# RemoteSensingTools/vSmartMOM.jl

Hardware: AMD Instinct MI355X
Metric: spectral-points/s (whole node) for rt_run, O2-A band (higher is better)
Workload: dtype f64; 1 GPU; C2: O2-A 759-770 nm, nStokes=3, Nquad=20 (N=60), 40 layers, 10000 spectral points/GPU, m=0..2, Rayleigh+synthetic O2 absorption, Lambertian 0.15; ranks=1, collective_backend=none (1 rank), N=60, layers=40, points_per_gpu=10000, fourier_moments=3

## Files before the change

include/vsmartmom_hip.h:

```cpp
#ifndef VSMARTMOM_HIP_H
#define VSMARTMOM_HIP_H

#include <stddef.h>
#include <stdint.h>

#ifdef __cplusplus
extern "C" {
#endif

typedef enum vsm_status {
  VSM_OK = 0,
  VSM_ERR_INVALID_ARG = 1,
  VSM_ERR_UNSUPPORTED = 2,
  VSM_ERR_HIP = 3,
  VSM_ERR_NO_DEVICE = 4
} vsm_status;

typedef enum vsm_iface {
  VSM_IFACE_00 = 0,
  VSM_IFACE_01 = 1,
  VSM_IFACE_10 = 2,
  VSM_IFACE_11 = 3
} vsm_iface;

// ... 392 lines not shown
                      const double* F0, int ncomp, const double* const* Zpp, const double* const* Zmp, long long z_stride,
                      const double* fcomp, int toa, const int* layer_coupling_h, void* stream);
int vsm_run_layer_f32(vsm_run* run, int ndoubl, const float* dtau, const float* varpi, const float* tau_sum,
                      const float* F0, int ncomp, const float* const* Zpp, const float* const* Zmp, long long z_stride,
                      const float* fcomp, int toa, const int* layer_coupling_h, void* stream);
int vsm_run_export_f64(vsm_run* run, const vsm_composite_f64* comps, void* stream);
int vsm_run_export_f32(vsm_run* run, const vsm_composite_f32* comps, void* stream);
int vsm_run_import_f64(vsm_run* run, const vsm_composite_f64* comps, void* stream);
int vsm_run_import_f32(vsm_run* run, const vsm_composite_f32* comps, void* stream);
int vsm_run_zw_tail(vsm_run* run);
int vsm_run_view_rows(vsm_run* run, int nrows, const int* rows_h);
int vsm_run_view_block(const vsm_run* run, int block, int* im, int* n, int* nv, int* local_rows);
int vsm_run_view_rows(vsm_run* run, int nrows, const int* rows_h);
int vsm_run_view_block(const vsm_run* run, int block, int* im, int* n, int* nv, int* local_rows);
int vsm_run_destroy(vsm_run* run);
int vsm_stokes_coupling_f64(int N, int n_stokes, int nblocks, const double* Zpp, const double* Zmp, int* mask_d, void* stream);
int vsm_stokes_coupling_f32(int N, int n_stokes, int nblocks, const float* Zpp, const float* Zmp, int* mask_d, void* stream);

typedef struct vsm_added_rs_f64 {
  double *ier_mp, *iet_pp, *ier_pm, *iet_mm;
  double *ieJ0_p, *ieJ0_m;
  int K;
  int reserved;
} vsm_added_rs_f64;
typedef struct vsm_added_rs_f32 {
  float *ier_mp, *iet_pp, *ier_pm, *iet_mm;
  float *ieJ0_p, *ieJ0_m;
  int K;
  int reserved;
} vsm_added_rs_f32;
// ... 243 lines not shown
```

vsmartmom.jl_amd/_lib.py:

```python
from __future__ import annotations

import ctypes as C
import os

_HERE = os.path.dirname(os.path.abspath(__file__))
LIB_PATH = os.environ.get("VSM_LIB_PATH") or os.path.join(_HERE, "lib", "libvsmartmom_hip.so")


class VSMError(RuntimeError):
    pass


class vsm_quad_f64(C.Structure):
    _fields_ = [("mu", C.c_void_p), ("wt", C.c_void_p), ("N", C.c_int), ("n_stokes", C.c_int),
                ("i_mu0", C.c_int), ("mu0", C.c_double)]


class vsm_quad_f32(C.Structure):
    _fields_ = [("mu", C.c_void_p), ("wt", C.c_void_p), ("N", C.c_int), ("n_stokes", C.c_int),
                ("i_mu0", C.c_int), ("mu0", C.c_float)]


class vsm_added(C.Structure):
    _fields_ = [("r_mp", C.c_void_p), ("t_pp", C.c_void_p), ("r_pm", C.c_void_p), ("t_mm", C.c_void_p),
# ... 127 lines not shown
    "vsm_exact_ss_jac12_{T}": (_I, [_I, _I, _I, _I, _I, _P, _P, _P, _P, _I, _P, "{R}", _P, _P, _P, _P, _P, _P, _P]),
    "vsm_run_supported": (_I, [_I, _I, _I]),
    "vsm_run_workspace_bytes": (_SZ, [_I, _I, _I, _I, _P]),
    "vsm_run_supported_f32": (_I, [_I, _I, _I]),
    "vsm_run_workspace_bytes_f32": (_SZ, [_I, _I, _I, _I, _P]),
    "vsm_run_create_{T}": (_I, [_P, _I, _I, _P, _P, _P, _SZ, _P]),
    "vsm_run_create_ex_{T}": (_I, [_P, _I, _I, _P, _P, _P, _SZ, C.c_uint, _P]),
    "vsm_run_create_view_{T}": (_I, [_P, _I, _I, _P, _P, _P, _SZ, C.c_uint, _I, _P, _P]),
    "vsm_run_layer_{T}": (_I, [_P, _I, _P, _P, _P, _P, _I, _P, _P, _LL, _P, _I, _P, _P]),
    "vsm_run_export_{T}": (_I, [_P, _P, _P]),
    "vsm_run_import_{T}": (_I, [_P, _P, _P]),
    "vsm_run_zw_tail": (_I, [_P]),
    "vsm_run_view_rows": (_I, [_P, _I, _P]),
    "vsm_run_view_block": (_I, [_P, _I, _P, _P, _P, _P]),
    "vsm_run_destroy": (_I, [_P]),
    "vsm_stokes_coupling_{T}": (_I, [_I, _I, _I, _P, _P, _P, _P]),
    "vsm_level_radiance_work_elems": (_SZ, [_I, _I]),
    "vsm_level_radiance_{T}": (_I, [_I, _I, _I, _I, _P, _P, _P, _P, _P, _LL, _P, _P, _P, _P, _P, _P, _P]),
    "vsm_level_radiance_oplevel_{T}": (_I, [_I, _I, _I, _I, _P, _P, _P, _P, _P, _LL, _P, _P, _P, _P, _P, _P, _P]),
    "vsm_level_radiance_src_{T}": (_I, [_I, _I, _I, _I, _P, _P, _P, _I, _P, _P, _LL, _P, _P, _P, _P, _P, _P, _P]),
    "vsm_level_flux_{T}": (_I, [_I, _I, _I, _P, _I, _P, _P, _LL, _P, _I, _P, _P, "{R}", _P, _P, _P, _P]),
    "vsm_surface_emission_response_{T}": (_I, [_I, _I, _I, _I, _P, _I, _P, _P, _P, _P, _P, _LL, _P, _P, _P]),
    "vsm_level_radiance_ie_{T}": (_I, [_I, _I, _I, _I, _P, _I, _P, _P, _P, _P, _LL, _P, _P, _P, _P, _P, _P, _P, _P, _P, _P, _P]),
    "vsm_level_flux_ie_{T}": (_I, [_I, _I, _I, _I, _P, _P, _P, _LL, _P, _P, _P, _P, _P, _P, _I, _P, _P, "{R}", _P, _P, _P, _P]),
    "vsm_level_radiance_lin_{T}": (_I, [_I, _I, _I, _I, _I, _I, _P, _P, _P, _P, _LL, _P, _P, _P, _LL, _P, _P, _LL, _LL, _P, _P, _P, _P, _P,
                                        _P]),
    "vsm_level_radiance_lin_src_{T}": (_I, [_I, _I, _I, _I, _I, _I, _I, _P, _P, _P, _P, _LL, _P, _P, _P, _LL, _P, _P, _LL, _LL, _P, _P, _P,
                                            _P, _P, _P, _P, _P]),
    "vsm_level_flux_lin_{T}": (_I, [_I, _I, _I, _I, _I, _I, _P, _P, _LL, _P, _P, _P, _LL, _P, _P, _LL, _LL, _P, _P, _P, _I, _P, _P,
                                    "{R}", _P, _P, _P, _I, _P, _P]),
# ... 102 lines not shown
```

vsmartmom.jl_amd/core_rt.py:

```python
from __future__ import annotations

import contextlib
import ctypes as C
import dataclasses
import math
import os
import warnings
from dataclasses import dataclass
from typing import List, Optional

import numpy as np
import torch

from . import _lib
from . import host_model as H
from .architectures import GPU, CPU, architecture, array_type, devi, synchronize_if_gpu, to_host

IFACE = {"00": 0, "01": 1, "10": 2, "11": 3}
MOMENT_BATCH = 4
MOMENT_BATCH_MAX = 24
MOMENT_BATCHING = True
THERMAL_FUSION = True
NATIVE_RUN = True
NATIVE_SOURCES_ONLY = True
NATIVE_VIEW_ROWS = True
VIEW_ROWS_MAX = 16
NATIVE_ZW_TAIL = True
NATIVE_DROPIN = True
REFERENCE_ORDER = False


def _require_gpu(arch):
    if not isinstance(arch, GPU):
        raise _lib.VSMError("vsmartmom.jl_amd provides the MI355X path only; architecture %r has no compute path here "
                            "(no CPU fallback by design)" % (arch,))
    if not torch.cuda.is_available():
        raise _lib.VSMError("no MI355X visible to HIP (torch.cuda.is_available() is False)")
    if arch.device_index != torch.cuda.current_device():
        raise _lib.VSMError("architecture GPU(%d) is not the current HIP device (%d): one process per GPU -- call "
                            "torch.cuda.set_device(%d) first" % (arch.device_index, torch.cuda.current_device(),
                                                                 arch.device_index))

# ... 90 lines not shown
        self.d_symmetric = int(d_symmetric)
        self.r_pm, self.t_mm = (None, None) if self.d_symmetric else (z(), z())
        self.j0_p = torch.zeros((nSpec, N), dtype=dt, device=dev)
        self.j0_m = torch.zeros((nSpec, N), dtype=dt, device=dev)
        self.N, self.nSpec, self.shared, self.dtype = N, nSpec, shared, dt

    def cstruct(self):
        return _lib.vsm_added(self.r_mp.data_ptr(), self.t_pp.data_ptr(),
                              0 if self.r_pm is None else self.r_pm.data_ptr(),
                              0 if self.t_mm is None else self.t_mm.data_ptr(),
                              self.j0_p.data_ptr(), self.j0_m.data_ptr(), 0 if self.shared else self.N * self.N,
                              self.d_symmetric, 0)


def _composite_field(name):
    def fget(self):
        return self.materialize()._arr[name]

    def fset(self, value):
        self.materialize()._arr[name] = value
    return property(fget, fset)


class CompositeLayer:

    def __init__(self, FT, arch, N, nSpec):
        dev, dt = devi(arch), _torch_dtype(FT)
        z = lambda: torch.zeros((nSpec, N, N), dtype=dt, device=dev)
        self._native = None
        self._sources_only = False
        self._view_rows = None
        self._native_ws = None
        self._arr = dict(R_mp=z(), R_pm=z(), T_pp=z(), T_mm=z(), J0_p=torch.zeros((nSpec, N), dtype=dt, device=dev),
                         J0_m=torch.zeros((nSpec, N), dtype=dt, device=dev))
        self.N, self.nSpec, self.dtype = N, nSpec, dt

    R_mp, R_pm, T_pp = _composite_field("R_mp"), _composite_field("R_pm"), _composite_field("T_pp")
    T_mm, J0_p, J0_m = _composite_field("T_mm"), _composite_field("J0_p"), _composite_field("J0_m")

    def materialize(self):
        slot = self._native
        if slot is None:
            return self
        self._native = None
        try:
            cc = (_lib.vsm_composite * 1)(self._cstruct_raw())
            _lib.call("vsm_run_export", self.dtype, slot.run, cc, _stream_ptr())
        finally:
            _lib.lib().vsm_run_destroy(slot.run)
        return self

    def snapshot_top(self):
        slot = self._native
        if slot is not None:
            cc = (_lib.vsm_composite * 1)(self._cstruct_raw())
            _lib.call("vsm_run_export", self.dtype, slot.run, cc, _stream_ptr())
            a = self._arr
        else:
            a = self.materialize()._arr
        return a["R_pm"].clone(), a["J0_p"].clone()

    def drop_native(self):
        slot, self._native = self._native, None
        if slot is not None:
            _lib.lib().vsm_run_destroy(slot.run)

    def _cstruct_raw(self):
        a = self._arr
        return _lib.vsm_composite(a["R_mp"].data_ptr(), a["R_pm"].data_ptr(), a["T_pp"].data_ptr(), a["T_mm"].data_ptr(),
                                  a["J0_p"].data_ptr(), a["J0_m"].data_ptr())

    def cstruct(self):
        self.materialize()
        return self._cstruct_raw()

    def __del__(self):
        try:
            self.drop_native()
        except Exception:
            pass


def make_added_layer(FT, arch, dims, nSpec, shared=False, d_symmetric=0) -> AddedLayer:
    _require_gpu(arch)
    return AddedLayer(FT, arch, dims[0], nSpec, shared, d_symmetric)


def make_composite_layer(FT, arch, dims, nSpec) -> CompositeLayer:
    _require_gpu(arch)
# ... 149 lines not shown
def reflectance(surf, dq: DeviceQuad, m: int, arch, FT, deriv: bool = False):
    if isinstance(surf, (H.rpvSurfaceScalar, H.RossLiSurfaceScalar)):
        if deriv:
            raise _lib.VSMError("%s has no linearization (types.jl:472-512)" % type(surf).__name__)
        return to_device_matrix(H.brdf_reflectance(surf, dq.n_stokes, dq.host.qp_mu.astype(np.float64), m), arch, FT)[0].contiguous(), None
    N = int(dq.mu.numel())
    rho = torch.empty((N, N), dtype=dq.dtype, device=dq.mu.device)
    drho = torch.empty_like(rho) if deriv else None
    phi, w = brdf_azimuth_quadrature(arch, FT)
    cs, q = _coxmunk_cstruct(surf, dq.dtype), dq.cstruct()
    _lib.call("vsm_coxmunk_reflectance", dq.dtype, C.byref(cs), C.byref(q), m, int(phi.numel()), _ptr(phi), _ptr(w), _ptr(rho),
              _ptr(drho), _stream_ptr())
    return rho, drho


def create_surface_layer_(surface, added_surface: AddedLayer, m: int, dq: DeviceQuad, tau_sum: torch.Tensor, rho=None,
                          arch=None, FT=None):
    q, a = dq.cstruct(), added_surface.cstruct()
    if isinstance(surface, (H.LambertianSurfaceLegendre, H.LambertianSurfaceSpline)):
        if added_surface.shared or rho is None:
            raise _lib.VSMError("spectral Lambertian surfaces need a per-point surface AddedLayer and their albedo spectrum")
        _lib.call("vsm_lambertian_surface_spectral", added_surface.dtype, C.byref(q), added_surface.nSpec, m, _ptr(rho),
                  _ptr(tau_sum), C.byref(a), _stream_ptr())
        return
    if not added_surface.shared:
        raise _lib.VSMError("surface AddedLayer must be allocated with shared=True")
    if isinstance(surface, H.LambertianSurfaceScalar):
        surface = surface.albedo
    if isinstance(surface, (int, float)):
        alb = C.c_double(surface) if added_surface.dtype == torch.float64 else C.c_float(surface)
        _lib.call("vsm_lambertian_surface", added_surface.dtype, C.byref(q), added_surface.nSpec, m, alb, _ptr(tau_sum),
                  C.byref(a), _stream_ptr())
        return
    if isinstance(surface, BRDF_SURFACES):
        if rho is None:
            rho, _ = reflectance(surface, dq, m, arch, FT)
        _lib.call("vsm_brdf_surface", added_surface.dtype, C.byref(q), added_surface.nSpec, m, _ptr(rho), _ptr(tau_sum),
                  C.byref(a), _stream_ptr())
        return
    raise _lib.VSMError("surface %r is not built in this backend (LambertianSurfaceScalar / Legendre / Spline, CoxMunkSurface, "
                        "rpvSurfaceScalar, RossLiSurfaceScalar)"
                        % (surface,))


SIF_SURFACES = (H.LambertianSurfaceScalar, H.LambertianSurfaceLegendre, H.LambertianSurfaceSpline)


def surface_source_contribute_(scene_or_table, surface, added_surface: AddedLayer, m: int) -> bool:
    scene = scene_or_table if isinstance(scene_or_table, Scene) else None
    table = scene.sif if scene is not None else scene_or_table
    if table is None or m != 0:
        return False
    if not isinstance(surface, SIF_SURFACES + (int, float)):
        if scene is None or not scene._sif_warned:
# ... 57 lines not shown
        for k in range(n):
            w[v + nV * k] = weight * [c, c, s, s][k]
    return row0, w


def postprocessing_vza_(pol: H.PolarizationType, comp: CompositeLayer, vza, vaz, qp: H.QuadPoints, m: int, weight: float,
                        R_SFI: torch.Tensor, T_SFI: torch.Tensor):
    n, nV = pol.n, len(vza)
    row0, w = _vza_rows_weights(pol, vza, vaz, qp, m, weight, comp.dtype)
    _lib.call("vsm_postprocess_vza", comp.dtype, comp.N, n, comp.nSpec, nV, row0, w, _ptr(comp.J0_m), _ptr(comp.J0_p),
              _ptr(R_SFI), _ptr(T_SFI), _stream_ptr())


def interaction_hdrf_(pol, comp: CompositeLayer, added_surface: AddedLayer, m: int, dq: DeviceQuad, vza, vaz, qp, weight: float,
                      hdr_J: torch.Tensor, hdr: torch.Tensor, bhr_uw: torch.Tensor, bhr_dw: torch.Tensor):
    q, c, a = dq.cstruct(), comp.cstruct(), added_surface.cstruct()
    _lib.call("vsm_interaction_hdrf", comp.dtype, C.byref(q), comp.nSpec, m, C.byref(c), C.byref(a), _ptr(hdr_J), _ptr(bhr_uw),
              _ptr(bhr_dw), _stream_ptr())
    row0, w = _vza_rows_weights(pol, vza, vaz, qp, m, weight, comp.dtype)
    _lib.call("vsm_postprocess_vza_hdrf", comp.dtype, comp.N, pol.n, comp.nSpec, len(vza), row0, w, _ptr(hdr_J), _ptr(hdr),
              _stream_ptr())


def init_layer(props: DeviceLayerOptics, qp: H.QuadPoints, FT, numerics: H.RTNumericalParameters, arch):
    dtau_h, nd = H.get_dtau_ndoubl(props.tau_h, props.varpi_h, qp, FT, numerics)
    return array_type(arch)(dtau_h), nd


@dataclass
class NativeSlot:
    run: C.c_void_p
    m: int
    coupling: int
    grp_of: List[int]


def stokes_groups(n_stokes: int, coupling: int) -> List[int]:
    adj = [[a == b or coupling < 0 or bool((coupling >> (4 * a + b)) & 1) or bool((coupling >> (4 * b + a)) & 1)
            for b in range(n_stokes)] for a in range(n_stokes)]
    grp = [-1] * n_stokes
    ng = 0
    for a in range(n_stokes):
        if grp[a] >= 0:
            continue
        grp[a], stack = ng, [a]
        while stack:
            x = stack.pop()
            for b in range(n_stokes):
                if adj[x][b] and grp[b] < 0:
# ... 53 lines not shown
    nbytes = run_workspace_bytes(comp.dtype, N, ns, S, 1, carr)
    ws = comp._native_ws
    if ws is None or ws.numel() * 8 < nbytes:
        ws = comp._native_ws = _lib.poison(torch.empty(max(nbytes // 8, 2), dtype=torch.float64, device=comp._arr["R_mp"].device))
    q = dq.cstruct()
    comp._native_q = (q, dq)
    run = C.c_void_p()
    run_create_(comp.dtype, q, S, 1, marr, carr, ws, nbytes, comp._sources_only, comp._view_rows, run)
    if import_arrays:
        try:
            cc = (_lib.vsm_composite * 1)(comp._cstruct_raw())
            _lib.call("vsm_run_import", comp.dtype, run, cc, _stream_ptr())
        except Exception:
            L.vsm_run_destroy(run)
            raise
    comp._native = NativeSlot(run, int(m), int(mask), stokes_groups(ns, mask))
    return True


def _rt_kernel_native(comp: CompositeLayer, props: DeviceLayerOptics, tau_sum, m: int, dq: DeviceQuad, iz: int, F0, dtau,
                      ndoubl: int) -> bool:
    N, ns, S = comp.N, dq.n_stokes, comp.nSpec
    ncomp = 0 if props.fcomp is None else int(props.fcomp.shape[1])
    if ncomp > 4 or S == 0:
        return False
    lc = layer_coupling(props, N, ns)
    if iz == 1:
        comp.drop_native()
        if not _native_open(comp, dq, m, lc, False):
            return False
    slot = comp._native
# ... 293 lines not shown
    def _layer_coupling(self, m, iz):
        mixed, k = self.zcomp[iz]
        row = self.coupling_comp[m]
        return int(np.bitwise_or.reduce(row)) if mixed else int(row[k])

    def run(self, trace: Optional[list] = None, streams: Optional[list] = None):
        model, pol, FT = self.model, self.pol, self.FT
        if self.layers_only:
            raise _lib.VSMError("Scene(layers_only=True) holds no composite layer: it feeds rt_run_ss only")
        self.R_SFI.zero_()
        self.T_SFI.zero_()
        self.hdr.zero_()
        if self.S == 0:
            return self.R_SFI, self.T_SFI
        self.added.j0_p.zero_()
        eps2 = 2 * np.finfo(FT).eps
        has_noscat = any(ly["props"].max_tau_varpi <= eps2 for ly in self.moments[0]["layers"])
        nb = self._group_size(trace is not None or not MOMENT_BATCHING or has_noscat or REFERENCE_ORDER)
        native = self._native_moments() if trace is None and not has_noscat and not REFERENCE_ORDER else set()
        walk_src = streams is None and trace is None and not has_noscat
        if getattr(self, "_view_rows", None) is None:
            self._view_rows = view_rows_of(pol, model.vza, self.qp)
        view_rows = self._view_rows if streams is None else None
        with self._walk_composites(nb, walk_src and REFERENCE_ORDER, view_rows):
            for g0 in range(0, len(self.moments), nb):
                group = self.moments[g0:g0 + nb]
                comps = self._composites[:len(group)]
                self._walk_layers(group, comps, [k for k in range(len(group)) if (g0 + k) in native], sources_only=streams is None,
                                  view_rows=view_rows, trace=trace, keep_added=has_noscat)
                for mom, comp in zip(group, comps):
                    m = mom["m"]
                    weight = float(fourier_weight(FT, m))
                    create_surface_layer_(model.surface, self.added_surface, m, self.dq, mom["tau_sum_surface"], rho=mom["rho"])
                    surface_source_contribute_(self, model.surface, self.added_surface, m)
                    interaction_(mom["iface_surface"], comp, self.added_surface, work=self.work)
                    if self.compute_hdrf:
                        interaction_hdrf_(pol, comp, self.added_surface, m, self.dq, model.vza, model.vaz, self.qp, weight,
                                          self.hdr_J, self.hdr, self.bhr_uw, self.bhr_dw)
                    postprocessing_vza_(pol, comp, model.vza, model.vaz, self.qp, m, weight, self.R_SFI, self.T_SFI)
                    thermal_pass = self.thermal_B is not None and (m == 0 or (m == 1 and self.thermal_slot().carry))
                    if thermal_pass:
                        self._thermal_slot(mom, weight)
                    if streams is not None:
                        Jm, Jp = comp.J0_m.clone(), comp.J0_p.clone()
                        if thermal_pass:
                            Jm += self._thermal.comp.J0_m
                            Jp += self._thermal.comp.J0_p
                        streams.append(dict(m=m, weight=weight, R_mp=comp.R_mp.clone(), T_pp=comp.T_pp.clone(), J0_m=Jm, J0_p=Jp))
        if isinstance(model.surface, H.CoxMunkSurface) and self.ss_correction:
            apply_ss_correction_(self.R_SFI, model.surface, pol, model.vza, model.vaz, self.qp.mu0,
                                 self.moments[-1]["tau_sum_surface"], model.m_max, self.arch, FT)
        return self.R_SFI, self.T_SFI

    def _group_size(self, sequential: bool) -> int:
        want = max(MOMENT_BATCH, min(MOMENT_BATCH_MAX, 4096 // max(self.S, 1)))
        return 1 if sequential else min(want, len(self.moments))

    @contextlib.contextmanager
    def _walk_composites(self, nb: int, sources_only: bool, view_rows):
        while len(self._composites) < nb:
            self._composites.append(make_composite_layer(self.FT, self.arch, (self.N, self.N), self.S))
        for c in self._composites:
            c._sources_only = bool(sources_only)
            c._view_rows = view_rows if sources_only else None
        try:
            yield
        finally:
            for c in self._composites:
                c._sources_only = False
                c._view_rows = None

    def _walk_layers(self, group, comps, nat, sources_only: bool, view_rows, trace=None, keep_added: bool = False, tops_at=(),
                     keep_top=None):
        eps2 = 2 * np.finfo(self.FT).eps
        if nat:
            def export(l):
                def cb(cs):
                    for k, c in zip(nat, cs):
                        keep_top(k, l, (c._arr["R_pm"].clone(), c._arr["J0_p"].clone()))
                return cb
            self._run_layers_native([group[k] for k in nat], [comps[k] for k in nat], sources_only=sources_only,
                                    export_at={l: export(l) for l in tops_at}, view_rows=view_rows)
        rest = [k for k in range(len(group)) if k not in nat]
        group_l, comps_l = [group[k] for k in rest], [comps[k] for k in rest]
        for iz in range(self.Nz if rest else 0):
            ly0 = group_l[0]["layers"][iz]
            if len(group_l) > 1 and ly0["props"].max_tau_varpi > eps2 and (iz == 0 or ly0["iface"] == "11"):
                layer_forward_multi_(ly0["tau_sum"], ly0["dtau"], self.F0, [mom["layers"][iz]["props"] for mom in group_l],
                                     [mom["m"] for mom in group_l], ly0["nd"], self.dq, iz == 0, comps_l, self.added)
            else:
                for mom, comp in zip(group_l, comps_l):
                    ly = mom["layers"][iz]
                    rt_kernel_(self.pol, self.added, comp, ly["props"], ly["iface"], ly["tau_sum"], mom["m"], self.dq, self.arch,
                               iz + 1, self.F0, self.FT, self.model.numerics, dtau=ly["dtau"], ndoubl=ly["nd"], trace=trace,
                               work=self.work, keep_added=keep_added)
            if iz + 1 in tops_at:
                for k, comp in zip(rest, comps_l):
                    keep_top(k, iz + 1, comp.snapshot_top())

    def _native_moments(self):
        if not NATIVE_RUN or getattr(self, "coupling", None) is None or not self.moments:
            return set()
        eps2 = 2 * np.finfo(self.FT).eps
        for iz, ly in enumerate(self.moments[0]["layers"]):
            p = ly["props"]
            if p.max_tau_varpi <= eps2 or (iz > 0 and ly["iface"] != "11") or (p.fcomp is not None and p.fcomp.shape[1] > 4):
                return set()
        return {i for i, mom in enumerate(self.moments) if run_supported(self.dt, self.N, self.pol.n, int(self.coupling[mom["m"]]))}

    def _run_layers_native(self, group, comps, sources_only: bool = True, export_at=None, view_rows=None):
        L = _lib.lib()
        nm, N, S, ns = len(group), self.N, self.S, self.pol.n
        marr = (C.c_int * nm)(*[int(mom["m"]) for mom in group])
        carr = (C.c_int * nm)(*[int(self.coupling[mom["m"]]) for mom in group])
        nbytes = run_workspace_bytes(self.dt, N, ns, S, nm, carr)
        ws = getattr(self, "_native_ws", None)
        if ws is None or ws.numel() * 8 < nbytes:
            ws = self._native_ws = _lib.poison(torch.empty(max(nbytes // 8, 2), dtype=torch.float64, device=self.dev))
        q = self.dq.cstruct()
        run = C.c_void_p()
        run_create_(self.dt, q, S, nm, marr, carr, ws, nbytes, sources_only, view_rows, run)
        try:
            if NATIVE_ZW_TAIL and not torch.cuda.is_current_stream_capturing():
                _lib.check(L.vsm_run_zw_tail(run))
            for iz in range(self.Nz):
                ly0 = group[0]["layers"][iz]
                props = [mom["layers"][iz]["props"] for mom in group]
                p0 = props[0]
                zpp = (C.c_void_p * nm)(*[p.Zpp.data_ptr() for p in props])
                zmp = (C.c_void_p * nm)(*[p.Zmp.data_ptr() for p in props])
                ncomp = 0 if p0.fcomp is None else int(p0.fcomp.shape[1])
                lc = (C.c_int * nm)(*[self._layer_coupling(mom["m"], iz) for mom in group])
                run_layer_native_(run, nm, int(ly0["nd"]), ly0["dtau"], p0.varpi, ly0["tau_sum"], self.F0, ncomp, zpp, zmp,
                                  0 if ncomp else p0.z_stride, p0.fcomp, iz == 0, lc, self.dt)
                if export_at and (iz + 1) in export_at:
                    cc = (type(comps[0].cstruct()) * nm)(*[c.cstruct() for c in comps])
                    _lib.call("vsm_run_export", self.dt, run, cc, _stream_ptr())
                    export_at[iz + 1](comps)
            cc = (type(comps[0].cstruct()) * nm)(*[c.cstruct() for c in comps])
            _lib.call("vsm_run_export", self.dt, run, cc, _stream_ptr())
        finally:
            L.vsm_run_destroy(run)

    def thermal_slot(self) -> "ThermalSlot":
        if self._thermal is None:
            self._thermal = ThermalSlot(self)
        return self._thermal

    def _thermal_slot(self, mom, weight):
        th = self.thermal_slot()
        th.begin(mom)
        th.walk(mom, th.comp, 0, self.Nz, self.thermal_B)
        th.surface(mom)
        th.finish(mom, weight, self.R_SFI, self.T_SFI)

    def run_graph(self):
        if getattr(self, "_graph", None) is None:
# ... 168 lines not shown
```

vsmartmom.jl_amd/csrc/vsm_native.hip:

```cpp
#include <stdlib.h>

#include <vector>

#include "vsm_native_dev.h"
#include "vsm_native_run.h"

#ifndef VSM_NATIVE_PARK_RT
#define VSM_NATIVE_PARK_RT 3
#endif

namespace vsm {

struct nlayer_comps {
  double* c[NSUB_MAX];
};

namespace {

template <int RT, int KS, int KZ = KS, bool TILE = false>
__device__ __forceinline__ void ned_body(nsmem<RT, (4 * KS + 2 > 16 * RT)>& sm, npos<RT>& p, int n, int gsz, unsigned uvmask, int ndoubl,
                                         const double* __restrict__ img, nstrip<RT>& r_s, nstrip<RT>& t_s, int* status) {
  using G = ngeo<RT>;
  constexpr unsigned dP = 0, dQ = G::AF * 8;
  double* jp = sm.vec[0];
// ... 1235 lines not shown
    if (src) v[NC_RMP] = v[NC_TPP] = (T)__builtin_nan("");
    if (view && at < 0) v[NC_TMM] = (T)__builtin_nan("");
#pragma unroll
    for (int k = 0; k < 4; ++k) out[k][e] = v[k];
  }
  if (tid < N) {
    const int ai = tid % ns, gi = gm.grp_of[ai];
    const int rt = gm.rt[gi], np = 16 * rt, af = np * np;
    const T* cn = gm.base[gi] + (long long)s * (4 * af + 2 * np);
    const int is = (tid / ns) * gm.gsz[gi] + gm.pos_in[ai];
    c.J0_p[(long long)s * N + tid] = cn[4 * af + is];
    c.J0_m[(long long)s * N + tid] = (view && vw.find(gi, is) < 0) ? (T)__builtin_nan("") : cn[4 * af + np + is];
  }
}
template <typename T>
__global__ __launch_bounds__(256) void k_native_import(int N, int ns, int view, ngroup_map<T> gm, nview vw, composite<T> c) {
  const int s = blockIdx.x, tid = threadIdx.x;
  const long long NN = (long long)N * N;
  const T* in[4] = {c.R_mp + s * NN, c.R_pm + s * NN, c.T_pp + s * NN, c.T_mm + s * NN};
  for (int g = 0; g < gm.ngroups; ++g) {
    const int rt = gm.rt[g], np = 16 * rt, af = np * np, n = gm.n[g], gsz = gm.gsz[g];
    T* cn = gm.base[g] + (long long)s * (4 * af + 2 * np);
    int comp_of[4] = {0, 0, 0, 0};
    for (int a = 0; a < ns; ++a)
      if (gm.grp_of[a] == g) comp_of[gm.pos_in[a]] = a;
    for (int e = tid; e < af; e += 256) {
      const int is = e % np, js = e / np;
      T v[4] = {0, 0, 0, 0};
      if (is < n && js < n) {
        const int i = (is / gsz) * ns + comp_of[is % gsz], j = (js / gsz) * ns + comp_of[js % gsz];
// ... 438 lines not shown
  VSM_REQUIRE(run->elem_size == (int)sizeof(T), "vsm_run_layer: the run was created for %d-byte arrays", run->elem_size);
  VSM_REQUIRE(ndoubl >= 0 && ndoubl < 60 && ncomp >= 0 && ncomp <= 4 && (ncomp == 0 || fcomp), "vsm_run_layer: bad ndoubl / component mix");
  ++run->layers;
  if (run->S == 0) return VSM_OK;
  hipStream_t st = as_stream(stream);
  int* status = device_status();
  if (!status) return VSM_ERR_HIP;
  const quad<T> q = run_quad<T>(run);
  auto trivial = [&](const nat_sub& sb) {
    if (!layer_coupling || layer_coupling[sb.im] < 0) return false;
    for (int a = 0; a < sb.gsz; ++a)
      for (int b = 0; b < sb.gsz; ++b)
        if ((layer_coupling[sb.im] >> (4 * sb.g[a] + sb.g[b])) & 1) return false;
    return true;
  };
  {
    nguard_args<T> ga;
    for (int k = 0; k < NSUB_MAX; ++k) {
      const int im = k < run->nm ? k : 0;
      VSM_REQUIRE(Zpp[im] && Zmp[im], "vsm_run_layer: null Z of moment %d", im);
      ga.zp[k] = Zpp[im];
      ga.zm[k] = Zmp[im];
      ga.allowed[k] = 0;
    }
    for (const nat_sub& sb : run->subs) {
      if (trivial(sb)) continue;
      for (int a = 0; a < sb.gsz; ++a)
        for (int b = 0; b < sb.gsz; ++b) ga.allowed[sb.im] |= 1u << (4 * sb.g[a] + sb.g[b]);
    }
    const int nmat = ncomp ? ncomp : (z_stride ? run->S : 1);
    hipLaunchKernelGGL((k_coupling_guard<T>), dim3(nmat, run->nm), dim3(256), 0, st, run->N, run->ns,
                       ncomp ? (long long)run->N * run->N : z_stride, ga, status);
    VSM_LAUNCH_CHECK("k_coupling_guard");
  }
  T* const ws = static_cast<T*>(run->ws);
  const int src = (run->flags & VSM_RUN_SOURCES_ONLY) ? 1 : 0;
  const int view = (run->flags & VSM_RUN_VIEW_ROWS) ? 1 : 0;
  size_t pre_total = 0;
  for (const nat_sub& sb : run->subs)
    if (!trivial(sb)) pre_total += pre_stride_rt(sb.rt) * (size_t)run->S;
  T* pre = nullptr;
  if (pre_total) {
    pre = static_cast<T*>(scratch(pre_total * sizeof(T), 3, st));
    if (!pre) return VSM_ERR_HIP;
  }
  size_t off = 0;
  for (const auto& cl : run->classes) {
    const nat_sub& h = run->subs[cl[0]];
// ... 45 lines not shown
    if (rc) return rc;
  }
  return VSM_OK;
}

template <typename T, typename CS, bool IMPORT>
static int run_convert(vsm_run* run, const CS* comps, void* stream) {
  VSM_REQUIRE(run && comps, "vsm_run_export / import: null argument");
  VSM_REQUIRE(run->elem_size == (int)sizeof(T), "vsm_run_export / import: the run was created for %d-byte arrays", run->elem_size);
  if (IMPORT) ++run->imports;
  if (run->S == 0) return VSM_OK;
  if (IMPORT) {
    run->pure_diag.assign(run->subs.size(), 0);
    run->flags &= ~(unsigned)VSM_RUN_ZW_TAIL;
    for (nat_sub& sb : run->subs) sb.kz = sb.ks;
  }
  for (int im = 0; im < run->nm; ++im) {
    const CS& c = comps[im];
    VSM_REQUIRE(c.R_mp && c.R_pm && c.T_pp && c.T_mm && c.J0_p && c.J0_m, "vsm_run_export / import: null composite array (moment %d)", im);
    const composite<T> cc{c.R_mp, c.R_pm, c.T_pp, c.T_mm, c.J0_p, c.J0_m};
    const ngroup_map<T> gm = group_map<T>(run, im);
    const int view = (run->flags & VSM_RUN_VIEW_ROWS) ? 1 : 0;
    const nview vw = view ? view_of_moment(run, im) : nview{};
    if (IMPORT)
      hipLaunchKernelGGL((k_native_import<T>), dim3(run->S), dim3(256), 0, as_stream(stream), run->N, run->ns, view, gm, vw, cc);
    else
      hipLaunchKernelGGL((k_native_export<T>), dim3(run->S), dim3(256), 0, as_stream(stream), run->N, run->ns,
                         (run->flags & VSM_RUN_SOURCES_ONLY) ? 1 : 0, view, gm, vw, cc);
    VSM_LAUNCH_CHECK("k_native_export / import");
  }
  return VSM_OK;
}

template <typename T>
static int stokes_coupling(int N, int n_stokes, int nblocks, const T* Zpp, const T* Zmp, int* mask_d, void* stream) {
  VSM_REQUIRE(N > 0 && n_stokes >= 1 && n_stokes <= 4 && N % n_stokes == 0 && nblocks >= 1 && nblocks <= 65535 && Zpp && Zmp &&
                  mask_d, "vsm_stokes_coupling: bad argument");
  hipStream_t st = as_stream(stream);
  VSM_HIP(hipMemsetAsync(mask_d, 0, sizeof(int) * nblocks, st));
  const long long tot = (long long)N * N;
  const int blocks = (int)((tot + 255) / 256 < 16 ? (tot + 255) / 256 : 16);
  hipLaunchKernelGGL((k_stokes_coupling<T>), dim3(blocks, nblocks), dim3(256), 0, st, N, n_stokes, Zpp, Zmp, mask_d);
  VSM_LAUNCH_CHECK("k_stokes_coupling");
  return VSM_OK;
}

// ... 100 lines not shown
}

int vsm_run_export_f64(vsm_run* run, const vsm_composite_f64* comps, void* stream) {
  return run_convert<double, vsm_composite_f64, false>(run, comps, stream);
}
int vsm_run_export_f32(vsm_run* run, const vsm_composite_f32* comps, void* stream) {
  return run_convert<float, vsm_composite_f32, false>(run, comps, stream);
}
int vsm_run_import_f64(vsm_run* run, const vsm_composite_f64* comps, void* stream) {
  return run_convert<double, vsm_composite_f64, true>(run, comps, stream);
}
int vsm_run_import_f32(vsm_run* run, const vsm_composite_f32* comps, void* stream) {
  return run_convert<float, vsm_composite_f32, true>(run, comps, stream);
}

int vsm_stokes_coupling_f64(int N, int n_stokes, int nblocks, const double* Zpp, const double* Zmp, int* mask_d, void* stream) {
  return stokes_coupling<double>(N, n_stokes, nblocks, Zpp, Zmp, mask_d, stream);
}
int vsm_stokes_coupling_f32(int N, int n_stokes, int nblocks, const float* Zpp, const float* Zmp, int* mask_d, void* stream) {
  return stokes_coupling<float>(N, n_stokes, nblocks, Zpp, Zmp, mask_d, stream);
}

}

#endif
```

vsmartmom.jl_amd/csrc/vsm_native_run.h:

```cpp
#pragma once
#include <vector>

#include "vsm_internal.h"

namespace vsm {

constexpr int NSUB_MAX = VSM_MM_MAX;

struct nat_sub {
  int im;
  int m;
  int gsz, g[4];
  unsigned uvmask;
  int n, rt, ks;
  int kz;
  size_t comp_off;
  int nv;
  int vrow[VSM_RUN_VIEW_MAX];
};

struct nview {
  int nv[NSUB_MAX];
  unsigned pk[NSUB_MAX][VSM_RUN_VIEW_MAX / 4];
  __host__ __device__ int row(int k, int v) const { return (int)((pk[k][v >> 2] >> (8 * (v & 3))) & 255u); }
// ... 10 lines not shown
  const void *mu, *wt;
  int N, ns, i_mu0;
  double mu0;
  int elem_size;
  int S, nm;
  unsigned flags;
  std::vector<int> view_rows;
  std::vector<int> m;
  std::vector<vsm::nat_sub> subs;
  std::vector<std::vector<int>> classes;
  void* ws;
  size_t ws_elems;
  int layers = 0;
  int imports = 0;
  std::vector<char> pure_diag;
};

namespace vsm {

constexpr int NATIVE_MAX_ROWS = 96;
constexpr int NATIVE32_MAX_ROWS = 128;

constexpr int rt_of(int n) {
  const int ks = (n + 3) / 4;
  return (ks % 4 == 0 && ks >= 4) ? ks / 4 : (4 * ks + 2 + 15) / 16;
}
constexpr size_t comp_stride_rt(int rt) { return (size_t)4 * (16 * rt) * (16 * rt) + 2 * 16 * rt; }
constexpr size_t pre_stride_rt(int rt) { return (size_t)2 * (16 * rt) * (16 * rt) + 3 * 16 * rt; }

template <typename T>
// ... 18 lines not shown
```

vsmartmom.jl_amd/csrc/vsm_surface.hip:

```cpp
#include "vsm_internal.h"

namespace vsm {

template <typename T>
struct cplx {
  T re, im;
};
template <typename T>
__device__ __forceinline__ cplx<T> cmul(cplx<T> a, cplx<T> b) {
  return {a.re * b.re - a.im * b.im, a.re * b.im + a.im * b.re};
}
template <typename T>
__device__ __forceinline__ cplx<T> cdiv(cplx<T> a, cplx<T> b) {
  const T d = b.re * b.re + b.im * b.im;
  return {(a.re * b.re + a.im * b.im) / d, (a.im * b.re - a.re * b.im) / d};
}
template <typename T>
__device__ __forceinline__ cplx<T> csqrt(cplx<T> z) {
  const T r = sqrt(z.re * z.re + z.im * z.im);
  if (r == T(0)) return {T(0), T(0)};
  if (z.re >= T(0)) {
    const T a = sqrt((r + z.re) / 2);
    return {a, z.im / (2 * a)};
  }
// ... 892 lines not shown
                                   const added<T>&, const added_lin<T>&, hipStream_t);                                        \
  template int land_brdf_reflectance_lin<T>(int, const T*, int, int, const T*, int, int, const T*, const T*, T*, T*,          \
                                            hipStream_t);                                                                   \
  template int brdf_surface_lin_multi<T>(const quad<T>&, int, int, const T*, const T*, int, int, const T*, const T*, int,     \
                                         const T*, const added<T>&, const added_lin<T>&, hipStream_t);                      \
  template int interaction_hdrf<T>(const quad<T>&, int, int, const composite<T>&, const added<T>&, T*, T*, T*, hipStream_t);  \
  template int postprocess_vza_hdrf<T>(int, int, int, int, const int*, const T*, const T*, T*, hipStream_t);                  \
  template int coxmunk_ss_correction<T>(const cm_surf<T>&, int, int, int, const T*, const T*, T, int, int, const T*, const T*, \
                                        const T*, T*, T*, hipStream_t);                                                      \
  template int coxmunk_first_column<T>(const cm_surf<T>&, int, int, const T*, const T*, T, int, int, const T*, const T*, T*,  \
                                       T*, hipStream_t);
VSM_INST_SURF(double)
VSM_INST_SURF(float)

}
```

Baseline: 26750 spectral-points/s.

## Keep native run alive per moment; skip identity Lambertian surface interactions and repeated guards

Native layer runs are no longer exported and destroyed right after the layer walk. Each composite keeps a reference-counted handle to the run and exports lazily per moment. For a scalar Lambertian surface at m>=1 with no surface source the surface layer is an identity, so only the J0 source vectors are exported and the full matrix export plus interaction are skipped. The coupling-guard kernel also runs only on the first layer step. In exchange this adds lifetime and refcount complexity, counters, and a risk of stale or NaN vectors if the lazy state is mishandled.

```diff
diff --git a/include/vsmartmom_hip.h b/include/vsmartmom_hip.h
--- a/include/vsmartmom_hip.h
+++ b/include/vsmartmom_hip.h
@@ -430,6 +430,19 @@
 int vsm_run_view_rows(vsm_run* run, int nrows, const int* rows_h);
 int vsm_run_view_block(const vsm_run* run, int block, int* im, int* n, int* nv, int* local_rows);
 int vsm_run_destroy(vsm_run* run);
+enum { VSM_SURFACE_LAMBERTIAN_SCALAR = 0, VSM_SURFACE_LAMBERTIAN_SPECTRAL = 1, VSM_SURFACE_BRDF = 2 };
+enum { VSM_SURFACE_LAYER_IDENTITY = 1 };
+unsigned vsm_surface_layer_flags(int kind, int m, int has_surface_source);
+int vsm_run_export_moment_f64(vsm_run* run, int im, const vsm_composite_f64* comp, void* stream);
+int vsm_run_export_moment_f32(vsm_run* run, int im, const vsm_composite_f32* comp, void* stream);
+int vsm_run_export_sources_f64(vsm_run* run, int im, const vsm_composite_f64* comp, void* stream);
+int vsm_run_export_sources_f32(vsm_run* run, int im, const vsm_composite_f32* comp, void* stream);
+int vsm_run_surface_f64(vsm_run* run, int im, int iface, const vsm_added_f64* added_surface, int identity, int matrices,
+                        const vsm_composite_f64* comp, double* work, void* stream);
+int vsm_run_surface_f32(vsm_run* run, int im, int iface, const vsm_added_f32* added_surface, int identity, int matrices,
+                        const vsm_composite_f32* comp, float* work, void* stream);
+int vsm_run_guard_once(vsm_run* run);
+int vsm_run_counters(const vsm_run* run, int* counts_h);
 int vsm_stokes_coupling_f64(int N, int n_stokes, int nblocks, const double* Zpp, const double* Zmp, int* mask_d, void* stream);
 int vsm_stokes_coupling_f32(int N, int n_stokes, int nblocks, const float* Zpp, const float* Zmp, int* mask_d, void* stream);
 
diff --git a/vsmartmom.jl_amd/_lib.py b/vsmartmom.jl_amd/_lib.py
--- a/vsmartmom.jl_amd/_lib.py
+++ b/vsmartmom.jl_amd/_lib.py
@@ -165,6 +165,12 @@
     "vsm_run_view_rows": (_I, [_P, _I, _P]),
     "vsm_run_view_block": (_I, [_P, _I, _P, _P, _P, _P]),
     "vsm_run_destroy": (_I, [_P]),
+    "vsm_surface_layer_flags": (C.c_uint, [_I, _I, _I]),
+    "vsm_run_export_moment_{T}": (_I, [_P, _I, _P, _P]),
+    "vsm_run_export_sources_{T}": (_I, [_P, _I, _P, _P]),
+    "vsm_run_surface_{T}": (_I, [_P, _I, _I, _P, _I, _I, _P, _P, _P]),
+    "vsm_run_guard_once": (_I, [_P]),
+    "vsm_run_counters": (_I, [_P, _P]),
     "vsm_stokes_coupling_{T}": (_I, [_I, _I, _I, _P, _P, _P, _P]),
     "vsm_level_radiance_work_elems": (_SZ, [_I, _I]),
     "vsm_level_radiance_{T}": (_I, [_I, _I, _I, _I, _P, _P, _P, _P, _P, _LL, _P, _P, _P, _P, _P, _P, _P]),
diff --git a/vsmartmom.jl_amd/core_rt.py b/vsmartmom.jl_amd/core_rt.py
--- a/vsmartmom.jl_amd/core_rt.py
+++ b/vsmartmom.jl_amd/core_rt.py
@@ -26,6 +26,7 @@
 NATIVE_VIEW_ROWS = True
 VIEW_ROWS_MAX = 16
 NATIVE_ZW_TAIL = True
+NATIVE_IDENTITY_SURFACE = True
 NATIVE_DROPIN = True
 REFERENCE_ORDER = False
 
@@ -146,12 +147,38 @@
 
 
 def _composite_field(name):
+    vector = name in ("J0_p", "J0_m")
+
     def fget(self):
+        if vector and self._vectors_current:
+            return self._arr[name]
         return self.materialize()._arr[name]
 
     def fset(self, value):
         self.materialize()._arr[name] = value
     return property(fget, fset)
+
+
+RUN_COUNTERS = ("exports_full", "exports_src", "surface_interactions", "guard_launches")
+
+
+class RunRef:
+
+    def __init__(self, run, sink=None, keep=None, refs: int = 1):
+        self.run, self.sink, self.keep, self.refs = run, sink, keep, refs
+
+    def release(self):
+        self.refs -= 1
+        if self.refs == 0 and self.run is not None:
+            run, self.run = self.run, None
+            L = _lib.lib()
+            if self.sink is not None:
+                counts = (C.c_int * 4)()
+                if L.vsm_run_counters(run, counts) == 0:
+                    for k, v in zip(RUN_COUNTERS, counts):
+                        self.sink[k] = self.sink.get(k, 0) + int(v)
+            L.vsm_run_destroy(run)
+            self.keep = None
 
 
 class CompositeLayer:
@@ -163,6 +190,8 @@
         self._sources_only = False
         self._view_rows = None
         self._native_ws = None
+        self._vectors_current = False
+        self._counters = None
         self._arr = dict(R_mp=z(), R_pm=z(), T_pp=z(), T_mm=z(), J0_p=torch.zeros((nSpec, N), dtype=dt, device=dev),
                          J0_m=torch.zeros((nSpec, N), dtype=dt, device=dev))
         self.N, self.nSpec, self.dtype = N, nSpec, dt
@@ -174,28 +203,42 @@
         slot = self._native
         if slot is None:
             return self
-        self._native = None
+        self._native, self._vectors_current = None, False
         try:
-            cc = (_lib.vsm_composite * 1)(self._cstruct_raw())
-            _lib.call("vsm_run_export", self.dtype, slot.run, cc, _stream_ptr())
+            cc = self._cstruct_raw()
+            _lib.call("vsm_run_export_moment", self.dtype, slot.run, slot.im, C.byref(cc), _stream_ptr())
         finally:
-            _lib.lib().vsm_run_destroy(slot.run)
+            slot.ref.release()
         return self
+
+    def surface_step(self, iface: str, added_surface: "AddedLayer", identity: bool, matrices: bool, work) -> bool:
+        slot = self._native
+        if slot is None:
+            return False
+        a, cc = added_surface.cstruct(), self._cstruct_raw()
+        _lib.call("vsm_run_surface", self.dtype, slot.run, slot.im, IFACE[iface], C.byref(a), int(identity), int(matrices),
+                  C.byref(cc), _ptr(work), _stream_ptr())
+        if identity and not matrices:
+            self._vectors_current = True
+        else:
+            self._native = None
+            slot.ref.release()
+        return True
 
     def snapshot_top(self):
         slot = self._native
         if slot is not None:
-            cc = (_lib.vsm_composite * 1)(self._cstruct_raw())
-            _lib.call("vsm_run_export", self.dtype, slot.run, cc, _stream_ptr())
+            cc = self._cstruct_raw()
+            _lib.call("vsm_run_export_moment", self.dtype, slot.run, slot.im, C.byref(cc), _stream_ptr())
             a = self._arr
         else:
             a = self.materialize()._arr
         return a["R_pm"].clone(), a["J0_p"].clone()
 
     def drop_native(self):
-        slot, self._native = self._native, None
+        slot, self._native, self._vectors_current = self._native, None, False
         if slot is not None:
-            _lib.lib().vsm_run_destroy(slot.run)
+            slot.ref.release()
 
     def _cstruct_raw(self):
         a = self._arr
@@ -205,6 +248,9 @@
     def cstruct(self):
         self.materialize()
         return self._cstruct_raw()
+
+    def cstruct_sources(self):
+        return self._cstruct_raw() if self._vectors_current else self.cstruct()
 
     def __del__(self):
         try:
@@ -384,15 +430,23 @@
     return rho, drho
 
 
+SURFACE_LAMBERTIAN_SCALAR, SURFACE_LAMBERTIAN_SPECTRAL, SURFACE_BRDF = 0, 1, 2
+SURFACE_LAYER_IDENTITY = 1
+
+
+def surface_layer_flags(kind: int, m: int, has_surface_source: bool = False) -> int:
+    return int(_lib.lib().vsm_surface_layer_flags(int(kind), int(m), 1 if has_surface_source else 0))
+
+
 def create_surface_layer_(surface, added_surface: AddedLayer, m: int, dq: DeviceQuad, tau_sum: torch.Tensor, rho=None,
-                          arch=None, FT=None):
+                          arch=None, FT=None, has_surface_source: bool = False) -> int:
     q, a = dq.cstruct(), added_surface.cstruct()
     if isinstance(surface, (H.LambertianSurfaceLegendre, H.LambertianSurfaceSpline)):
         if added_surface.shared or rho is None:
             raise _lib.VSMError("spectral Lambertian surfaces need a per-point surface AddedLayer and their albedo spectrum")
         _lib.call("vsm_lambertian_surface_spectral", added_surface.dtype, C.byref(q), added_surface.nSpec, m, _ptr(rho),
                   _ptr(tau_sum), C.byref(a), _stream_ptr())
-        return
+        return surface_layer_flags(SURFACE_LAMBERTIAN_SPECTRAL, m, has_surface_source)
     if not added_surface.shared:
         raise _lib.VSMError("surface AddedLayer must be allocated with shared=True")
     if isinstance(surface, H.LambertianSurfaceScalar):
@@ -401,13 +455,13 @@
         alb = C.c_double(surface) if added_surface.dtype == torch.float64 else C.c_float(surface)
         _lib.call("vsm_lambertian_surface", added_surface.dtype, C.byref(q), added_surface.nSpec, m, alb, _ptr(tau_sum),
                   C.byref(a), _stream_ptr())
-        return
+        return surface_layer_flags(SURFACE_LAMBERTIAN_SCALAR, m, has_surface_source)
     if isinstance(surface, BRDF_SURFACES):
         if rho is None:
             rho, _ = reflectance(surface, dq, m, arch, FT)
         _lib.call("vsm_brdf_surface", added_surface.dtype, C.byref(q), added_surface.nSpec, m, _ptr(rho), _ptr(tau_sum),
                   C.byref(a), _stream_ptr())
-        return
+        return surface_layer_flags(SURFACE_BRDF, m, has_surface_source)
     raise _lib.VSMError("surface %r is not built in this backend (LambertianSurfaceScalar / Legendre / Spline, CoxMunkSurface, "
                         "rpvSurfaceScalar, RossLiSurfaceScalar)"
                         % (surface,))
@@ -495,7 +549,7 @@
 
 def interaction_hdrf_(pol, comp: CompositeLayer, added_surface: AddedLayer, m: int, dq: DeviceQuad, vza, vaz, qp, weight: float,
                       hdr_J: torch.Tensor, hdr: torch.Tensor, bhr_uw: torch.Tensor, bhr_dw: torch.Tensor):
-    q, c, a = dq.cstruct(), comp.cstruct(), added_surface.cstruct()
+    q, c, a = dq.cstruct(), comp.cstruct_sources(), added_surface.cstruct()
     _lib.call("vsm_interaction_hdrf", comp.dtype, C.byref(q), comp.nSpec, m, C.byref(c), C.byref(a), _ptr(hdr_J), _ptr(bhr_uw),
               _ptr(bhr_dw), _stream_ptr())
     row0, w = _vza_rows_weights(pol, vza, vaz, qp, m, weight, comp.dtype)
@@ -514,6 +568,8 @@
     m: int
     coupling: int
     grp_of: List[int]
+    ref: RunRef = None
+    im: int = 0
 
 
 def stokes_groups(n_stokes: int, coupling: int) -> List[int]:
@@ -597,7 +653,7 @@
         except Exception:
             L.vsm_run_destroy(run)
             raise
-    comp._native = NativeSlot(run, int(m), int(mask), stokes_groups(ns, mask))
+    comp._native = NativeSlot(run, int(m), int(mask), stokes_groups(ns, mask), RunRef(run, comp._counters))
     return True
 
 
@@ -921,6 +977,8 @@
         if self.S == 0:
             return self.R_SFI, self.T_SFI
         self.added.j0_p.zero_()
+        self._drop_lazy()
+        self.__dict__.setdefault("_run_counts", {}).clear()
         eps2 = 2 * np.finfo(FT).eps
         has_noscat = any(ly["props"].max_tau_varpi <= eps2 for ly in self.moments[0]["layers"])
         nb = self._group_size(trace is not None or not MOMENT_BATCHING or has_noscat or REFERENCE_ORDER)
@@ -929,18 +987,23 @@
         if getattr(self, "_view_rows", None) is None:
             self._view_rows = view_rows_of(pol, model.vza, self.qp)
         view_rows = self._view_rows if streams is None else None
+        has_surface_source = self.sif is not None or self.surface_B is not None
         with self._walk_composites(nb, walk_src and REFERENCE_ORDER, view_rows):
             for g0 in range(0, len(self.moments), nb):
                 group = self.moments[g0:g0 + nb]
                 comps = self._composites[:len(group)]
                 self._walk_layers(group, comps, [k for k in range(len(group)) if (g0 + k) in native], sources_only=streams is None,
-                                  view_rows=view_rows, trace=trace, keep_added=has_noscat)
+                                  view_rows=view_rows, trace=trace, keep_added=has_noscat, keep_native=True)
                 for mom, comp in zip(group, comps):
                     m = mom["m"]
                     weight = float(fourier_weight(FT, m))
-                    create_surface_layer_(model.surface, self.added_surface, m, self.dq, mom["tau_sum_surface"], rho=mom["rho"])
-                    surface_source_contribute_(self, model.surface, self.added_surface, m)
-                    interaction_(mom["iface_surface"], comp, self.added_surface, work=self.work)
+                    flags = create_surface_layer_(model.surface, self.added_surface, m, self.dq, mom["tau_sum_surface"], rho=mom["rho"],
+                                                  has_surface_source=has_surface_source)
+                    if surface_source_contribute_(self, model.surface, self.added_surface, m):
+                        flags &= ~SURFACE_LAYER_IDENTITY
+                    identity = bool(flags & SURFACE_LAYER_IDENTITY) and NATIVE_IDENTITY_SURFACE and mom["iface_surface"] == "11"
+                    if not comp.surface_step(mom["iface_surface"], self.added_surface, identity, streams is not None, self.work):
+                        interaction_(mom["iface_surface"], comp, self.added_surface, work=self.work)
                     if self.compute_hdrf:
                         interaction_hdrf_(pol, comp, self.added_surface, m, self.dq, model.vza, model.vaz, self.qp, weight,
                                           self.hdr_J, self.hdr, self.bhr_uw, self.bhr_dw)
@@ -959,6 +1022,22 @@
                                  self.moments[-1]["tau_sum_surface"], model.m_max, self.arch, FT)
         return self.R_SFI, self.T_SFI
 
+    def _drop_lazy(self):
+        for c in self._composites:
+            if c._vectors_current:
+                c.drop_native()
+
+    def run_counters(self) -> dict:
+        tot = {k: 0 for k in RUN_COUNTERS}
+        tot.update(self.__dict__.get("_run_counts", {}))
+        live = {id(c._native.ref): c._native.ref for c in self._composites if c._native is not None}
+        for ref in live.values():
+            counts = (C.c_int * 4)()
+            _lib.check(_lib.lib().vsm_run_counters(ref.run, counts))
+            for k, v in zip(RUN_COUNTERS, counts):
+                tot[k] += int(v)
+        return tot
+
     def _group_size(self, sequential: bool) -> int:
         want = max(MOMENT_BATCH, min(MOMENT_BATCH_MAX, 4096 // max(self.S, 1)))
         return 1 if sequential else min(want, len(self.moments))
@@ -970,6 +1049,7 @@
         for c in self._composites:
             c._sources_only = bool(sources_only)
             c._view_rows = view_rows if sources_only else None
+            c._counters = self.__dict__.setdefault("_run_counts", {})
         try:
             yield
         finally:
@@ -978,7 +1058,7 @@
                 c._view_rows = None
 
     def _walk_layers(self, group, comps, nat, sources_only: bool, view_rows, trace=None, keep_added: bool = False, tops_at=(),
-                     keep_top=None):
+                     keep_top=None, keep_native: bool = False):
         eps2 = 2 * np.finfo(self.FT).eps
         if nat:
             def export(l):
@@ -987,7 +1067,7 @@
                         keep_top(k, l, (c._arr["R_pm"].clone(), c._arr["J0_p"].clone()))
                 return cb
             self._run_layers_native([group[k] for k in nat], [comps[k] for k in nat], sources_only=sources_only,
-                                    export_at={l: export(l) for l in tops_at}, view_rows=view_rows)
+                                    export_at={l: export(l) for l in tops_at}, view_rows=view_rows, keep_native=keep_native)
         rest = [k for k in range(len(group)) if k not in nat]
         group_l, comps_l = [group[k] for k in rest], [comps[k] for k in rest]
         for iz in range(self.Nz if rest else 0):
@@ -1015,8 +1095,9 @@
                 return set()
         return {i for i, mom in enumerate(self.moments) if run_supported(self.dt, self.N, self.pol.n, int(self.coupling[mom["m"]]))}
 
-    def _run_layers_native(self, group, comps, sources_only: bool = True, export_at=None, view_rows=None):
+    def _run_layers_native(self, group, comps, sources_only: bool = True, export_at=None, view_rows=None, keep_native: bool = False):
         L = _lib.lib()
+        self._drop_lazy()
         nm, N, S, ns = len(group), self.N, self.S, self.pol.n
         marr = (C.c_int * nm)(*[int(mom["m"]) for mom in group])
         carr = (C.c_int * nm)(*[int(self.coupling[mom["m"]]) for mom in group])
@@ -1027,7 +1108,9 @@
         q = self.dq.cstruct()
         run = C.c_void_p()
         run_create_(self.dt, q, S, nm, marr, carr, ws, nbytes, sources_only, view_rows, run)
+        ref = RunRef(run, self.__dict__.setdefault("_run_counts", {}), keep=(ws, self.dq))
         try:
+            _lib.check(L.vsm_run_guard_once(run))
             if NATIVE_ZW_TAIL and not torch.cuda.is_current_stream_capturing():
                 _lib.check(L.vsm_run_zw_tail(run))
             for iz in range(self.Nz):
@@ -1044,10 +1127,17 @@
                     cc = (type(comps[0].cstruct()) * nm)(*[c.cstruct() for c in comps])
                     _lib.call("vsm_run_export", self.dt, run, cc, _stream_ptr())
                     export_at[iz + 1](comps)
-            cc = (type(comps[0].cstruct()) * nm)(*[c.cstruct() for c in comps])
-            _lib.call("vsm_run_export", self.dt, run, cc, _stream_ptr())
+            if keep_native:
+                for im, (mom, c) in enumerate(zip(group, comps)):
+                    c.drop_native()
+                    mask = int(self.coupling[mom["m"]])
+                    c._native = NativeSlot(run, int(mom["m"]), mask, stokes_groups(ns, mask), ref, im)
+                    ref.refs += 1
+            else:
+                cc = (type(comps[0].cstruct()) * nm)(*[c.cstruct() for c in comps])
+                _lib.call("vsm_run_export", self.dt, run, cc, _stream_ptr())
         finally:
-            L.vsm_run_destroy(run)
+            ref.release()
 
     def thermal_slot(self) -> "ThermalSlot":
         if self._thermal is None:
diff --git a/vsmartmom.jl_amd/csrc/vsm_native.hip b/vsmartmom.jl_amd/csrc/vsm_native.hip
--- a/vsmartmom.jl_amd/csrc/vsm_native.hip
+++ b/vsmartmom.jl_amd/csrc/vsm_native.hip
@@ -1273,6 +1273,19 @@
   }
 }
 template <typename T>
+__global__ __launch_bounds__(256) void k_native_export_src(int N, int ns, int S, int view, ngroup_map<T> gm, nview vw, T* __restrict__ J0_p,
+                                                           T* __restrict__ J0_m) {
+  const long long e = blockIdx.x * 256ll + threadIdx.x;
+  if (e >= (long long)S * N) return;
+  const int s = (int)(e / N), i = (int)(e % N);
+  const int ai = i % ns, gi = gm.grp_of[ai];
+  const int rt = gm.rt[gi], np = 16 * rt, af = np * np;
+  const T* cn = gm.base[gi] + (long long)s * (4 * af + 2 * np);
+  const int is = (i / ns) * gm.gsz[gi] + gm.pos_in[ai];
+  J0_p[e] = cn[4 * af + is];
+  J0_m[e] = (view && vw.find(gi, is) < 0) ? (T)__builtin_nan("") : cn[4 * af + np + is];
+}
+template <typename T>
 __global__ __launch_bounds__(256) void k_native_import(int N, int ns, int view, ngroup_map<T> gm, nview vw, composite<T> c) {
   const int s = blockIdx.x, tid = threadIdx.x;
   const long long NN = (long long)N * N;
@@ -1741,7 +1754,7 @@
         if ((layer_coupling[sb.im] >> (4 * sb.g[a] + sb.g[b])) & 1) return false;
     return true;
   };
-  {
+  if (!run->guard_once || run->layers == 1) {
     nguard_args<T> ga;
     for (int k = 0; k < NSUB_MAX; ++k) {
       const int im = k < run->nm ? k : 0;
@@ -1759,6 +1772,7 @@
     hipLaunchKernelGGL((k_coupling_guard<T>), dim3(nmat, run->nm), dim3(256), 0, st, run->N, run->ns,
                        ncomp ? (long long)run->N * run->N : z_stride, ga, status);
     VSM_LAUNCH_CHECK("k_coupling_guard");
+    ++run->guards;
   }
   T* const ws = static_cast<T*>(run->ws);
   const int src = (run->flags & VSM_RUN_SOURCES_ONLY) ? 1 : 0;
@@ -1834,6 +1848,7 @@
     run->pure_diag.assign(run->subs.size(), 0);
     run->flags &= ~(unsigned)VSM_RUN_ZW_TAIL;
     for (nat_sub& sb : run->subs) sb.kz = sb.ks;
+    run->guard_once = false;
   }
   for (int im = 0; im < run->nm; ++im) {
     const CS& c = comps[im];
@@ -1848,8 +1863,45 @@
       hipLaunchKernelGGL((k_native_export<T>), dim3(run->S), dim3(256), 0, as_stream(stream), run->N, run->ns,
                          (run->flags & VSM_RUN_SOURCES_ONLY) ? 1 : 0, view, gm, vw, cc);
     VSM_LAUNCH_CHECK("k_native_export / import");
+    if (!IMPORT) ++run->exports_full;
   }
   return VSM_OK;
+}
+
+template <typename T, typename CS>
+static int run_export_moment(vsm_run* run, int im, const CS* c, bool full, void* stream, const char* who) {
+  VSM_REQUIRE(run && c, "%s: null argument", who);
+  VSM_REQUIRE(run->elem_size == (int)sizeof(T), "%s: the run was created for %d-byte arrays", who, run->elem_size);
+  VSM_REQUIRE(im >= 0 && im < run->nm, "%s: moment index %d outside the run's %d moments", who, im, run->nm);
+  VSM_REQUIRE(c->J0_p && c->J0_m && (!full || (c->R_mp && c->R_pm && c->T_pp && c->T_mm)), "%s: null composite array", who);
+  if (run->S == 0) return VSM_OK;
+  const ngroup_map<T> gm = group_map<T>(run, im);
+  const int view = (run->flags & VSM_RUN_VIEW_ROWS) ? 1 : 0;
+  const nview vw = view ? view_of_moment(run, im) : nview{};
+  if (full) {
+    const composite<T> cc{c->R_mp, c->R_pm, c->T_pp, c->T_mm, c->J0_p, c->J0_m};
+    hipLaunchKernelGGL((k_native_export<T>), dim3(run->S), dim3(256), 0, as_stream(stream), run->N, run->ns,
+                       (run->flags & VSM_RUN_SOURCES_ONLY) ? 1 : 0, view, gm, vw, cc);
+    VSM_LAUNCH_CHECK("k_native_export");
+    ++run->exports_full;
+  } else {
+    const long long tot = (long long)run->S * run->N;
+    hipLaunchKernelGGL((k_native_export_src<T>), dim3((unsigned)((tot + 255) / 256)), dim3(256), 0, as_stream(stream), run->N, run->ns,
+                       run->S, view, gm, vw, c->J0_p, c->J0_m);
+    VSM_LAUNCH_CHECK("k_native_export_src");
+    ++run->exports_src;
+  }
+  return VSM_OK;
+}
+
+template <typename T, typename CS, typename AS>
+static int run_surface(vsm_run* run, int im, int iface, const AS* added_surface, int identity, int matrices, const CS* comp, T* work,
+                       void* stream, int (*interaction)(int, int, int, const CS*, const AS*, T*, void*)) {
+  VSM_REQUIRE(run && comp && (identity || added_surface), "vsm_run_surface: null argument");
+  const int rc = run_export_moment<T>(run, im, comp, !identity || matrices, stream, "vsm_run_surface");
+  if (rc || identity) return rc;
+  ++run->surface_ia;
+  return interaction(iface, run->N, run->S, comp, added_surface, work, stream);
 }
 
 template <typename T>
@@ -1980,6 +2032,44 @@
   return run_convert<float, vsm_composite_f32, true>(run, comps, stream);
 }
 
+int vsm_run_export_moment_f64(vsm_run* run, int im, const vsm_composite_f64* comp, void* stream) {
+  return run_export_moment<double>(run, im, comp, true, stream, "vsm_run_export_moment");
+}
+int vsm_run_export_moment_f32(vsm_run* run, int im, const vsm_composite_f32* comp, void* stream) {
+  return run_export_moment<float>(run, im, comp, true, stream, "vsm_run_export_moment");
+}
+int vsm_run_export_sources_f64(vsm_run* run, int im, const vsm_composite_f64* comp, void* stream) {
+  return run_export_moment<double>(run, im, comp, false, stream, "vsm_run_export_sources");
+}
+int vsm_run_export_sources_f32(vsm_run* run, int im, const vsm_composite_f32* comp, void* stream) {
+  return run_export_moment<float>(run, im, comp, false, stream, "vsm_run_export_sources");
+}
+
+int vsm_run_surface_f64(vsm_run* run, int im, int iface, const vsm_added_f64* added_surface, int identity, int matrices,
+                        const vsm_composite_f64* comp, double* work, void* stream) {
+  return run_surface<double>(run, im, iface, added_surface, identity, matrices, comp, work, stream, vsm_interaction_f64);
+}
+int vsm_run_surface_f32(vsm_run* run, int im, int iface, const vsm_added_f32* added_surface, int identity, int matrices,
+                        const vsm_composite_f32* comp, float* work, void* stream) {
+  return run_surface<float>(run, im, iface, added_surface, identity, matrices, comp, work, stream, vsm_interaction_f32);
+}
+
+int vsm_run_guard_once(vsm_run* run) {
+  VSM_REQUIRE(run, "vsm_run_guard_once: null argument");
+  VSM_REQUIRE(run->layers == 0 && run->imports == 0, "vsm_run_guard_once: the run has taken layer steps or an import already");
+  run->guard_once = true;
+  return VSM_OK;
+}
+
+int vsm_run_counters(const vsm_run* run, int* counts) {
+  VSM_REQUIRE(run && counts, "vsm_run_counters: null argument");
+  counts[0] = run->exports_full;
+  counts[1] = run->exports_src;
+  counts[2] = run->surface_ia;
+  counts[3] = run->guards;
+  return VSM_OK;
+}
+
 int vsm_stokes_coupling_f64(int N, int n_stokes, int nblocks, const double* Zpp, const double* Zmp, int* mask_d, void* stream) {
   return stokes_coupling<double>(N, n_stokes, nblocks, Zpp, Zmp, mask_d, stream);
 }
diff --git a/vsmartmom.jl_amd/csrc/vsm_native_run.h b/vsmartmom.jl_amd/csrc/vsm_native_run.h
--- a/vsmartmom.jl_amd/csrc/vsm_native_run.h
+++ b/vsmartmom.jl_amd/csrc/vsm_native_run.h
@@ -48,6 +48,8 @@
   int layers = 0;
   int imports = 0;
   std::vector<char> pure_diag;
+  bool guard_once = false;
+  int exports_full = 0, exports_src = 0, surface_ia = 0, guards = 0;
 };
 
 namespace vsm {
diff --git a/vsmartmom.jl_amd/csrc/vsm_surface.hip b/vsmartmom.jl_amd/csrc/vsm_surface.hip
--- a/vsmartmom.jl_amd/csrc/vsm_surface.hip
+++ b/vsmartmom.jl_amd/csrc/vsm_surface.hip
@@ -930,3 +930,8 @@
 VSM_INST_SURF(float)
 
 }
+
+extern "C" unsigned vsm_surface_layer_flags(int kind, int m, int has_surface_source) {
+  if (kind == VSM_SURFACE_LAMBERTIAN_SCALAR && m >= 1 && !has_surface_source) return VSM_SURFACE_LAYER_IDENTITY;
+  return 0u;
+}
```

Measured after the change: 27050 spectral-points/s, median of 6. 1.1% higher.
